# pytorch/QNNPACK

Hardware: AMD Instinct MI355X
Metric: q8gemm_int8_tops (higher is better)
Workload: dtype u8; 1 GPU; q8gemm M=N=K=4096 uint8 (qnnp_fully_connected_nc_q8, int8 MFMA, fused Q31 requantize); kernel=q8_gemm_mfma_256x256_c16, device=gfx950:sramecc+:xnack-, compute_units=256

## Files before the change

### qnnpack_amd/csrc/hip/q8gemm256x.hip

```cpp
#include <hip/hip_runtime.h>

#include <stdint.h>
#include <stdlib.h>

#include <type_traits>

#include "device_ops.hip.h"
#include "gemm256x_map.h"
#include "igemm_params.h"
#include "per_device.h"
#include "requant.hip.h"

namespace qnnp {

namespace {

namespace map = g256x;

constexpr int kBM = 256;
constexpr int kBN = 256;
constexpr int kBK = 64;
constexpr int kThreads = 512;
constexpr int kTM = 4;
constexpr int kTN = 8;
constexpr int kHalf = kTN / 2;
constexpr int kMma = kTM * kHalf;
static_assert(kBM == map::kRows && kBK == map::kTileK && kThreads == map::kWgThreads, "gemm256x_map.h describes this tile");

template <int P1, bool P2, int SYNC, bool MORE>
struct Tile {
  static constexpr int p1 = P1;
  static constexpr bool p2 = P2;
  static constexpr int sync = SYNC;
  static constexpr bool more = MORE;
};
constexpr int kSlotsEven = 0, kSlotsOdd = 1, kSlotsLiteral = 2;
using FirstTile = Tile<1, true, map::kFirstVmcnt, true>;
using SteadyTile = Tile<1, true, map::kSteadyVmcnt, true>;
template <bool ODD, uint32_t LEFT>
using DrainTile = Tile<map::p1_mode(ODD, LEFT), map::p2_issues(LEFT), map::sync_vmcnt(ODD, LEFT), LEFT != 1>;

template <int SEQ, int CLAMP, int SLOTS, int ABL = 0, bool ROWSUM = false, int OPT = 0>
__global__ __launch_bounds__(kThreads, 2)
void q8_gemm_mfma_256x256_c16_kernel(const IgemmParams p)
{
  static_assert(SEQ == kRqShift0Ofs || SEQ == kRqBoundedOfs || SEQ == kRqGeneral, "offset forms, or the general one");
  __shared__ __attribute__((aligned(16))) uint8_t lds[map::kLdsBytes];

  const uint32_t tid = threadIdx.x;
  const uint32_t lane = tid & 63u;
  const uint32_t wave = __builtin_amdgcn_readfirstlane(tid >> 6);
  const uint32_t wm = wave >> 1;
  const uint32_t wn = wave & 1u;
  const uint32_t g = blockIdx.y;
  QNNP_TRACE_WAVE04(p, lane, wave, 0);
  QNNP_TRACE_WAVE04_WALL(p, lane, wave, 0);

  const uint32_t tiles_m = (p.rows + kBM - 1) / kBM;
  const uint32_t tiles_n = p.n_pad / kBN;
  uint32_t m_tile, n_tile;
  {
    const uint32_t nwg = gridDim.x;
    const uint32_t xcd = blockIdx.x & 7u;
    const uint32_t idx = blockIdx.x >> 3;
    const uint32_t q = nwg >> 3, r = nwg & 7u;
    const uint32_t logical = xcd * q + min(xcd, r) + idx;
    constexpr uint32_t kBand = 4;
    const uint32_t band = p.tiles_n_magic != 0 ? __umulhi(logical >> 2, p.tiles_n_magic) : logical >> 2;
    const uint32_t within = logical - band * kBand * tiles_n;
    const uint32_t rows_in_band = min(kBand, tiles_m - band * kBand);
    if (rows_in_band == kBand) {
      m_tile = band * kBand + (within & 3u);
      n_tile = within >> 2;
    } else {
      m_tile = band * kBand + within % rows_in_band;
      n_tile = within / rows_in_band;
    }
  }

  const uint32_t nblocks = p.n_pad / 32;
  const uint32_t kblocks = p.k_pad / 32;
  const uint32_t ktiles = p.k_pad / kBK;
  const uint32_t nb0 = n_tile * (kBN / 32);

  const bool table_rows = p.offsets_dense != 0;
  const uint8_t* a_base = scalar_ptr(table_rows ? p.input + static_cast<uint64_t>(g) * p.kc
      : p.input + static_cast<uint64_t>(m_tile * kBM) * p.input_stride + static_cast<uint64_t>(g) * p.kc);
  uint32_t a_voff[map::kAPieces];
#pragma unroll
  for (uint32_t i = 0; i < map::kAPieces; i++) {
    const uint32_t m = map::a_clamp_row(m_tile * kBM + map::a_dma_row(i, tid), p.rows);
    a_voff[i] = (m - m_tile * kBM) * p.input_stride + map::a_dma_src(tid, false);
    if (table_rows) {
      const uint32_t img = p.rpi_magic != 0 ? __umulhi(m, p.rpi_magic) : m / p.rows_per_image;
      const uint32_t pix = m - img * p.rows_per_image;
      a_voff[i] = img * static_cast<uint32_t>(p.image_stride) + static_cast<uint32_t>(p.offsets[pix]) + map::a_dma_src(tid, false);
    }
  }
  const uint32_t a_half_back = map::a_dma_src(tid, false) - map::a_dma_src(tid, true);
  const uint8_t* w_base = scalar_ptr(reinterpret_cast<const uint8_t*>(p.packed_w) + static_cast<uint64_t>(g) * nblocks * kblocks * 1024 +
      (static_cast<uint64_t>(nb0 + (wave >> 1)) * kblocks + (wave & 1u)) * 1024);
  uint32_t w_voff[2];
#pragma unroll
  for (int i = 0; i < 2; i++) w_voff[i] = lane * 16 + static_cast<uint32_t>(i) * 4u * kblocks * 1024u;

  auto a_dst = [&](uint32_t piece, uint32_t slot) __attribute__((always_inline)) -> uint8_t* {
    return lds + map::kABase + slot * map::kPairBytes + map::a_dma_wave_dst(piece, wave);
  };
  auto w_dst = [&](uint32_t piece, uint32_t slot) __attribute__((always_inline)) -> uint8_t* {
    return lds + map::kWBase + slot * map::kWTileBytes + (piece * 8 + wave) * 1024;
  };
  auto a_src = [&](uint32_t pair) __attribute__((always_inline)) -> const uint8_t* {
    return a_base + static_cast<uint64_t>(pair) * map::kPairK;
  };
  auto w_src = [&](uint32_t kt) __attribute__((always_inline)) -> const uint8_t* {
    return w_base + static_cast<uint64_t>(kt) * 2048;
  };
  auto stage_pair = [&](uint32_t pair) __attribute__((always_inline)) {
#pragma unroll
    for (uint32_t piece = 0; piece < map::kAPieces; piece++) dma16_saddr(a_src(pair), a_voff[piece], a_dst(piece, map::a_slot(pair)));
  };
  auto stage_w = [&](uint32_t kt) __attribute__((always_inline)) {
#pragma unroll
    for (uint32_t piece = 0; piece < map::kWPieces; piece++) dma16_saddr(w_src(kt), w_voff[piece], w_dst(piece, map::w_slot(kt)));
  };

  stage_pair(0);
  stage_w(0);

  const int32_t* bias_tab = SEQ == kRqGeneral ? p.bias2 : p.bias2u;
  uint8_t* bias_line = lds + map::kBiasBase + wave * 512;
  if (lane < 32) {
    dma16_saddr(scalar_ptr(reinterpret_cast<const uint8_t*>(bias_tab + static_cast<uint64_t>(g) * p.n_pad + (nb0 + wn * 4) * 32)),
                   lane * 16, bias_line);
  }

  stage_pair(1);
  stage_w(1);
  stage_w(2);

  const uint32_t frow = lane & 15u;
  const uint32_t fg = lane >> 4;
  uint32_t a_off[2][2];
  uint32_t w_off;
#pragma unroll
  for (uint32_t h = 0; h < 2; h++) {
#pragma unroll
    for (uint32_t s2 = 0; s2 < 2; s2++) {
      a_off[h][s2] = map::kABase + map::a_lds_byte(map::a_frag_row(wm, 0, lane), map::a_frag_chunk(h, lane)) + s2 * 2 * map::kPairBytes;
      asm volatile("" : "+v"(a_off[h][s2]));
    }
  }
  w_off = map::kWBase + (wn * 8 + (fg >> 1)) * 1024 + (frow + 32 * (fg & 1u)) * 16;
  asm volatile("" : "+v"(w_off));
  v4i fa[kTM];
  v4i wl[kHalf], wh[kHalf];

  auto read_a = [&](auto known_c, uint32_t h, uint32_t slot, int tm) __attribute__((always_inline)) {
    const uint32_t imm = tm * 16 * map::kPairK;
    if constexpr (decltype(known_c)::value) {
      fa[tm] = *reinterpret_cast<const v4i*>(lds + a_off[h][slot >> 1] + (slot & 1u) * map::kPairBytes + imm);
    } else {
      fa[tm] = *reinterpret_cast<const v4i*>(lds + slot * map::kPairBytes + a_off[h][0] + imm);
    }
  };
  auto read_w = [&](auto known_c, uint32_t slot, int tn, v4i& dst) __attribute__((always_inline)) {
    const uint32_t imm = (tn >> 1) * 2048 + (tn & 1) * 256;
    dst = *reinterpret_cast<const v4i*>(lds + slot * map::kWTileBytes + w_off + imm);
  };

  const uint32_t flip = p.a_flip;
  uint32_t rs[kTM] = {0u, 0u, 0u, 0u};
  auto flip_half = [&](int tm, int half) __attribute__((always_inline)) {
    if constexpr (ROWSUM) {
      if (half) {
        rs[tm] = __builtin_amdgcn_sad_u8(static_cast<uint32_t>(fa[tm].z), 0u, rs[tm]);
        rs[tm] = __builtin_amdgcn_sad_u8(static_cast<uint32_t>(fa[tm].w), 0u, rs[tm]);
      } else {
        rs[tm] = __builtin_amdgcn_sad_u8(static_cast<uint32_t>(fa[tm].x), 0u, rs[tm]);
        rs[tm] = __builtin_amdgcn_sad_u8(static_cast<uint32_t>(fa[tm].y), 0u, rs[tm]);
      }
      asm volatile("" : "+v"(rs[tm]));
    }
    if constexpr ((ABL & 2) != 0) {
      asm volatile("" : "+v"(fa[tm]));
    } else if (half) {
      fa[tm].z ^= static_cast<int>(flip);
      fa[tm].w ^= static_cast<int>(flip);
      asm volatile("" : "+v"(fa[tm].z), "+v"(fa[tm].w));
    } else {
      fa[tm].x ^= static_cast<int>(flip);
      fa[tm].y ^= static_cast<int>(flip);
      asm volatile("" : "+v"(fa[tm].x), "+v"(fa[tm].y));
    }
  };

  v4i acc[kTM][kTN];
  auto mma = [&](const v4i& w, int tm, int tn) __attribute__((always_inline)) {
    if constexpr ((ABL & 4) != 0) return;
    acc[tm][tn] = __builtin_amdgcn_mfma_i32_16x16x64_i8(w, fa[tm], acc[tm][tn], 0, 0, 0);
  };

  wait_vmcnt<map::kPrologueVmcnt>();
  __builtin_amdgcn_s_barrier();
  QNNP_TRACE_WAVE04(p, lane, wave, 1);
  using T = std::true_type;
  using F = std::false_type;
#pragma unroll
  for (int tm = 0; tm < kTM; tm++) read_a(T{}, 0u, 0u, tm);
#pragma unroll
  for (int tn = 0; tn < kHalf; tn++) read_w(T{}, 0u, tn, wl[tn]);
#pragma unroll
  for (int tn = 0; tn < kTN; tn++) {
    const v4i b = *reinterpret_cast<const v4i*>(bias_line + tn * 64 + fg * 16);
#pragma unroll
    for (int tm = 0; tm < kTM; tm++) acc[tm][tn] = b;
  }
#pragma unroll
  for (int tm = 0; tm < 2; tm++) { flip_half(tm, 0); flip_half(tm, 1); }
  asm volatile("" : "+v"(wl[0]), "+v"(wl[1]), "+v"(wl[2]), "+v"(wl[3]));
  if constexpr ((ABL & 16) != 0) { wh[0] = wl[0]; wh[1] = wl[1]; wh[2] = wl[2]; wh[3] = wl[3]; }

  if constexpr ((OPT & 4) != 0) {
    if (wave >= 4) __builtin_amdgcn_s_setprio(1);
  }

  auto iteration = [&](auto tile_c, auto known_c, auto h_c, uint32_t kt, uint32_t ws, uint32_t as) __attribute__((always_inline)) {
    using TileT = decltype(tile_c);
    constexpr int P1 = (ABL & 8) != 0 ? 0 : TileT::p1;
    constexpr bool MORE = TileT::more;
    constexpr bool P2F = TileT::p2 && (ABL & 8) == 0;
    constexpr int SYNC = (ABL & 32) != 0 ? -1 : TileT::sync;
    constexpr bool KNOWN = decltype(known_c)::value;
    constexpr bool READS = (ABL & 16) == 0;
    constexpr uint32_t H = decltype(h_c)::value;
    const uint32_t ws_next = ws + 1 == map::kWSlots ? 0 : ws + 1;
    const uint32_t as_fill = as == 0 ? map::kASlots - 1 : as - 1;
    const uint32_t as_next = H == 0 ? as : (as + 1 == map::kASlots ? 0 : as + 1);
    auto a_piece_off = [&](uint32_t piece) __attribute__((always_inline)) -> uint32_t {
      return P1 == 2 ? a_voff[piece] - a_half_back : a_voff[piece];
    };

    QNNP_PIN();
#pragma unroll
    for (int i = 0; i < kMma; i++) {
      const int tm = i / kHalf, tn = ((OPT & 1) == 0 && (tm & 1) != 0) ? kHalf - 1 - i % kHalf : i % kHalf;
      if constexpr (P1 != 0 && KNOWN) {
        if (i % 8 == 0) { dma16_set_m0(a_dst(map::a_issue_piece(H, i / 8), as_fill)); QNNP_PIN(); }
      }
      mma(wl[tn], tm, tn);
      QNNP_PIN();
      if constexpr (READS) {
        if (i < kHalf) { read_w(known_c, ws, kHalf + i, wh[i]); QNNP_PIN(); }
      }
      if constexpr (P1 != 0 && KNOWN) {
        if (i % 8 == 0) { dma16_saddr_m0_set(a_src(map::a_issue_pair(kt)), a_piece_off(map::a_issue_piece(H, i / 8))); QNNP_PIN(); }
      } else if constexpr (P1 != 0) {
        if (i % 8 == 0) {
          dma16_saddr(a_src(map::a_issue_pair(kt)), a_piece_off(map::a_issue_piece(H, i / 8)), a_dst(map::a_issue_piece(H, i / 8), as_fill));
          QNNP_PIN();
        }
      }
      if (i == 2) { __builtin_amdgcn_s_waitcnt(0xC47F); QNNP_PIN(); }
      if (i == 2 || i == 3) { flip_half(2, i - 2); QNNP_PIN(); }
      if (i == 6) { __builtin_amdgcn_s_waitcnt(0xC47F); QNNP_PIN(); }
      if (i == 6 || i == 7) { flip_half(3, i - 6); QNNP_PIN(); }
      if (i == kMma - 2) { __builtin_amdgcn_s_waitcnt(0xC07F); QNNP_PIN(); }
    }
    asm volatile("" : "+v"(wh[0]), "+v"(wh[1]), "+v"(wh[2]), "+v"(wh[3]));
    QNNP_PIN();

    if constexpr (SYNC >= 0) {
      wait_vmcnt<SYNC>();
      __builtin_amdgcn_s_barrier();
    }
    QNNP_PIN();

#pragma unroll
    for (int i = 0; i < kMma; i++) {
      const int tm = i / kHalf, tn = ((OPT & 1) == 0 && (tm & 1) != 0) ? kHalf - 1 - i % kHalf : i % kHalf;
      if constexpr (P2F && KNOWN) {
        if (i % 8 == 0) { dma16_set_m0(w_dst(i / 8, ws)); QNNP_PIN(); }
      }
      mma(wh[tn], tm, kHalf + tn);
      QNNP_PIN();
      if constexpr (MORE && READS) {
        if (tm == 0) { read_w(known_c, ws_next, tn, wl[tn]); QNNP_PIN(); }
        if (i % kHalf == kHalf - 1) { read_a(known_c, 1u - H, as_next, tm); QNNP_PIN(); }
      }
      if constexpr (P2F && KNOWN) {
        if (i % 8 == 0) { dma16_saddr_m0_set(w_src(map::w_issue_tile(kt)), w_voff[i / 8]); QNNP_PIN(); }
      } else if constexpr (P2F) {
        if (i % 8 == 0) { dma16_saddr(w_src(map::w_issue_tile(kt)), w_voff[i / 8], w_dst(i / 8, ws)); QNNP_PIN(); }
      }
      if constexpr (MORE) {
        if (i == 9) { __builtin_amdgcn_s_waitcnt(0xC17F); QNNP_PIN(); }
        if (i == 9 || i == 10) { flip_half(0, i - 9); QNNP_PIN(); }
        if (i == 13) { __builtin_amdgcn_s_waitcnt(0xC17F); QNNP_PIN(); }
        if (i == 13 || i == 14) { flip_half(1, i - 13); QNNP_PIN(); }
      }
    }
    if constexpr (MORE) asm volatile("" : "+v"(wl[0]), "+v"(wl[1]), "+v"(wl[2]), "+v"(wl[3]));
    QNNP_PIN();
  };

  auto lit = [&](auto tile_c, auto x_c, uint32_t kt) __attribute__((always_inline)) {
    constexpr uint32_t X = decltype(x_c)::value;
    static_assert(X < map::kPeriod, "one ring period");
    iteration(tile_c, T{}, std::integral_constant<uint32_t, (X & 1u)>{}, kt, map::w_slot(X), map::a_slot(X >> 1));
  };
  using X0 = std::integral_constant<uint32_t, 0>;
  using X1 = std::integral_constant<uint32_t, 1>;
  using X2 = std::integral_constant<uint32_t, 2>;
  using X3 = std::integral_constant<uint32_t, 3>;
  using X4 = std::integral_constant<uint32_t, 4>;
  using X5 = std::integral_constant<uint32_t, 5>;

  lit(FirstTile{}, X0{}, 0u);
  QNNP_TRACE_WAVE04(p, lane, wave, 2);
  uint32_t kt = 1;
  if constexpr (SLOTS == kSlotsLiteral) {
    for (; kt + map::kPeriod + 4 + map::kDrain <= ktiles; kt += map::kPeriod) {
      lit(SteadyTile{}, X1{}, kt);
      lit(SteadyTile{}, X2{}, kt + 1);
      lit(SteadyTile{}, X3{}, kt + 2);
      lit(SteadyTile{}, X4{}, kt + 3);
      lit(SteadyTile{}, X5{}, kt + 4);
      lit(SteadyTile{}, X0{}, kt + 5);
    }
    lit(SteadyTile{}, X1{}, kt);
    lit(SteadyTile{}, X2{}, kt + 1);
    lit(SteadyTile{}, X3{}, kt + 2);
    lit(SteadyTile{}, X4{}, kt + 3);
    QNNP_TRACE_WAVE04(p, lane, wave, 3);
    lit(DrainTile<false, 5>{}, X5{}, kt + 4);
    lit(DrainTile<false, 4>{}, X0{}, kt + 5);
    lit(DrainTile<false, 3>{}, X1{}, kt + 6);
    QNNP_TRACE_WAVE04(p, lane, wave, 4);
    lit(DrainTile<false, 2>{}, X2{}, kt + 7);
    lit(DrainTile<false, 1>{}, X3{}, kt + 8);
  } else {
    uint32_t ws = 1, as = 0;
    using H0 = std::integral_constant<uint32_t, 0>;
    using H1 = std::integral_constant<uint32_t, 1>;
    auto odd_tile = [&](auto tile_c) __attribute__((always_inline)) {
      iteration(tile_c, F{}, H1{}, kt, ws, as);
      kt++;
      ws = ws + 1 == map::kWSlots ? 0 : ws + 1;
      as = as + 1 == map::kASlots ? 0 : as + 1;
    };
    auto even_tile = [&](auto tile_c) __attribute__((always_inline)) {
      iteration(tile_c, F{}, H0{}, kt, ws, as);
      kt++;
      ws = ws + 1 == map::kWSlots ? 0 : ws + 1;
    };
    while (kt + 1 + map::kDrain < ktiles) {
      odd_tile(SteadyTile{});
      even_tile(SteadyTile{});
    }
    QNNP_TRACE_WAVE04(p, lane, wave, 3);
    if constexpr (SLOTS == kSlotsOdd) {
      odd_tile(SteadyTile{});
      even_tile(DrainTile<true, 5>{});
      odd_tile(DrainTile<true, 4>{});
      even_tile(DrainTile<true, 3>{});
      odd_tile(DrainTile<true, 2>{});
      even_tile(DrainTile<true, 1>{});
    } else {
      odd_tile(DrainTile<false, 5>{});
      even_tile(DrainTile<false, 4>{});
      odd_tile(DrainTile<false, 3>{});
      even_tile(DrainTile<false, 2>{});
      odd_tile(DrainTile<false, 1>{});
    }
    QNNP_TRACE_WAVE04(p, lane, wave, 4);
  }
  QNNP_TRACE_WAVE04(p, lane, wave, 5);

  if constexpr ((ABL & 1) != 0) {
#pragma unroll
    for (int tm = 0; tm < kTM; tm++) {
#pragma unroll
      for (int tn = 0; tn < kTN; tn++) asm volatile("" : : "v"(acc[tm][tn]));
    }
    return;
  }
  const uint32_t m0 = m_tile * kBM + wm * 64;
  const uint32_t n0 = (nb0 + wn * 4) * 32;
  uint8_t* out0 = p.output + static_cast<uint64_t>(m0) * p.output_stride + static_cast<uint64_t>(g) * p.n + n0;
  const uint32_t st_row = frow & 7u;
  const uint32_t st_col = (frow >> 3) * 64 + fg * 16;
  const bool col_ok = n0 + st_col < p.n;
  auto transpose4 = [&](uint32_t (&q)[4]) __attribute__((always_inline)) {
    const auto s02 = __builtin_amdgcn_permlane32_swap(q[0], q[2], false, false);
    const auto s13 = __builtin_amdgcn_permlane32_swap(q[1], q[3], false, false);
    const auto lo = __builtin_amdgcn_permlane16_swap(s02[0], s13[0], false, false);
    const auto hi = __builtin_amdgcn_permlane16_swap(s02[1], s13[1], false, false);
    q[0] = lo[0]; q[1] = lo[1]; q[2] = hi[0]; q[3] = hi[1];
  };
#pragma unroll
  for (int tm = 0; tm < kTM; tm++) {
    if constexpr (ROWSUM) {
      uint32_t t = rs[tm];
      t += static_cast<uint32_t>(__shfl_xor(static_cast<int>(t), 16));
      t += static_cast<uint32_t>(__shfl_xor(static_cast<int>(t), 32));
      const uint32_t term = static_cast<uint32_t>(p.row_coeff) * (t - 128u * p.k_pad);
#pragma unroll
      for (int tn = 0; tn < kTN; tn++) {
#pragma unroll
        for (int r = 0; r < 4; r++) acc[tm][tn][r] = static_cast<int>(static_cast<uint32_t>(acc[tm][tn][r]) + term);
      }
    }
    uint32_t lo[4], hi[4];
#pragma unroll
    for (int j = 0; j < 4; j++) {
      lo[j] = q31_requantize_pack4_clamp<SEQ, CLAMP>(acc[tm][j][0], acc[tm][j][1], acc[tm][j][2], acc[tm][j][3], p.rq);
      hi[j] = q31_requantize_pack4_clamp<SEQ, CLAMP>(acc[tm][4 + j][0], acc[tm][4 + j][1], acc[tm][4 + j][2], acc[tm][4 + j][3], p.rq);
    }
    transpose4(lo);
    transpose4(hi);
    typedef int nt_v4i __attribute__((ext_vector_type(4)));
    nt_v4i x, y;
#pragma unroll
    for (int j = 0; j < 4; j++) {
      x[j] = __builtin_amdgcn_update_dpp(static_cast<int>(lo[j]), static_cast<int>(hi[j]), 0x128, 0xF, 0xC, false);
      y[j] = __builtin_amdgcn_update_dpp(static_cast<int>(hi[j]), static_cast<int>(lo[j]), 0x128, 0xF, 0x3, false);
    }
    const uint32_t rx = tm * 16 + st_row, ry = rx + 8;
    nt_v4i* dx = reinterpret_cast<nt_v4i*>(out0 + static_cast<uint64_t>(rx) * p.output_stride + st_col);
    nt_v4i* dy = reinterpret_cast<nt_v4i*>(out0 + static_cast<uint64_t>(ry) * p.output_stride + st_col);
    const bool stores = (ABL & 64) == 0 || p.rows == 0xFFFFFFFFu;
    if (m0 + rx < p.rows && col_ok && stores) {
      if (p.stream_out) asm volatile("global_store_dwordx4 %0, %1, off nt" : : "v"(dx), "v"(x) : "memory");
      else *dx = x;
    }
    if (m0 + ry < p.rows && col_ok && stores) {
      if (p.stream_out) asm volatile("global_store_dwordx4 %0, %1, off nt" : : "v"(dy), "v"(y) : "memory");
      else *dy = y;
    }
    if (tm == 1) QNNP_TRACE_WAVE04(p, lane, wave, 6);
  }
  QNNP_TRACE_WAVE04(p, lane, wave, 7);
#ifdef QNNP_ENABLE_ABLATION
  if (p.trace != nullptr) {
    wait_vmcnt<0>();
    QNNP_TRACE_WAVE04_WALL(p, lane, wave, 1);
  }
#endif
}
#undef QNNP_PIN

template <int SLOTS, bool ROWSUM>
int launch_x(const IgemmParams& p, const dim3& grid, hipStream_t stream)
{
  int rc = QNNP_HIP_EINVAL;
#ifdef QNNP_ENABLE_ABLATION
  if constexpr (SLOTS == kSlotsLiteral && !ROWSUM) {
    const char* env = getenv("QNNP_GFX950_ABLATE");
    const int abl = env != nullptr ? atoi(env) : 0;
#define QNNP_ABL_CASE(V) case V: hipLaunchKernelGGL((q8_gemm_mfma_256x256_c16_kernel<kRqShift0Ofs, 1, kSlotsLiteral, V>), grid, dim3(kThreads), 0, stream, p); \
        return launch_status();
    switch (abl) {
      QNNP_ABL_CASE(1) QNNP_ABL_CASE(2) QNNP_ABL_CASE(4) QNNP_ABL_CASE(8) QNNP_ABL_CASE(16) QNNP_ABL_CASE(24)
      QNNP_ABL_CASE(27) QNNP_ABL_CASE(32) QNNP_ABL_CASE(59) QNNP_ABL_CASE(64)
      default: break;
    }
#undef QNNP_ABL_CASE
    const char* oenv = getenv("QNNP_C16_OPT");
    if (oenv != nullptr && atoi(oenv) == 1) {
      hipLaunchKernelGGL((q8_gemm_mfma_256x256_c16_kernel<kRqShift0Ofs, 1, kSlotsLiteral, 0, false, 1>), grid, dim3(kThreads), 0, stream, p);
      return launch_status();
    }
    if (oenv != nullptr && atoi(oenv) == 4) {
      hipLaunchKernelGGL((q8_gemm_mfma_256x256_c16_kernel<kRqShift0Ofs, 1, kSlotsLiteral, 0, false, 4>), grid, dim3(kThreads), 0, stream, p);
      return launch_status();
    }
  }
#endif
  if (p.rq.f.shift != 0 && p.rq.f.bounded && p.rq.f.ofs_kind == 2 && !p.rq.full_range) {
    if (p.rq.zp_late == 0) hipLaunchKernelGGL((q8_gemm_mfma_256x256_c16_kernel<kRqBoundedOfs, 1, SLOTS, 0, ROWSUM>), grid, dim3(kThreads), 0, stream, p);
    else hipLaunchKernelGGL((q8_gemm_mfma_256x256_c16_kernel<kRqBoundedOfs, 2, SLOTS, 0, ROWSUM>), grid, dim3(kThreads), 0, stream, p);
    return launch_status();
  }
  requant_dispatch_ofs(p.rq, [&](auto seq, auto full) {
    constexpr int kSeq = decltype(seq)::value;
    if constexpr (decltype(full)::value) {
      hipLaunchKernelGGL((q8_gemm_mfma_256x256_c16_kernel<kSeq, 0, SLOTS, 0, ROWSUM>), grid, dim3(kThreads), 0, stream, p);
    } else if (p.rq.zp_late == 0) {
      hipLaunchKernelGGL((q8_gemm_mfma_256x256_c16_kernel<kSeq, 1, SLOTS, 0, ROWSUM>), grid, dim3(kThreads), 0, stream, p);
    } else {
      hipLaunchKernelGGL((q8_gemm_mfma_256x256_c16_kernel<kSeq, 2, SLOTS, 0, ROWSUM>), grid, dim3(kThreads), 0, stream, p);
    }
    rc = launch_status();
  });
  return rc;
}

}

int gemm256x_launch(const IgemmParams& p, uint32_t groups, hipStream_t stream, const char** name)
{
  const uint32_t tiles_m = (p.rows + kBM - 1) / kBM;
  const uint32_t tiles_n = p.n_pad / kBN;
  const dim3 grid(tiles_m * tiles_n, groups, 1);
  IgemmParams pm = p;
  pm.tiles_n_magic = tiles_n == 1 ? 0u : reciprocal_floor_plus1(tiles_n);
  const uint32_t ktiles = p.k_pad / kBK;
  const int slots = map::literal_slots(ktiles) ? kSlotsLiteral : (ktiles & 1u) != 0 ? kSlotsOdd : kSlotsEven;
  if (p.row_coeff != 0) {
    *name = "q8_gemm_mfma_256x256_r16";
    return slots == kSlotsLiteral ? launch_x<kSlotsLiteral, true>(pm, grid, stream)
         : slots == kSlotsOdd   ? launch_x<kSlotsOdd, true>(pm, grid, stream) : launch_x<kSlotsEven, true>(pm, grid, stream);
  }
  *name = "q8_gemm_mfma_256x256_c16";
  return slots == kSlotsLiteral ? launch_x<kSlotsLiteral, false>(pm, grid, stream)
       : slots == kSlotsOdd   ? launch_x<kSlotsOdd, false>(pm, grid, stream) : launch_x<kSlotsEven, false>(pm, grid, stream);
}

}
```

Baseline: 2816 TOPS.

## Split kernel arguments into hot/cold/table lines with explicit scalar loads

Replaces the IgemmParams kernel argument with a compact 192-byte struct laid out as a 64-byte hot header, a cold part and an offset table. Each part is fetched with explicit s_load instructions. The hot header is loaded up front; the cold part (output, requant params) is issued after the prologue DMAs and waited on later; the table is loaded only when indirect rows are used. The tile-index mapping replaces the modulo/divide path with a multiply-by-magic form. The goal is to cut kernel-entry scalar load latency and prologue stalls, at the cost of hand-written asm that must stay in sync with the struct layout.

```diff
diff --git a/qnnpack_amd/csrc/hip/gemm256x_args.h b/qnnpack_amd/csrc/hip/gemm256x_args.h
--- /dev/null
+++ b/qnnpack_amd/csrc/hip/gemm256x_args.h
@@ -0,0 +1,96 @@
+#pragma once
+
+#include <stddef.h>
+#include <stdint.h>
+
+#include "igemm_params.h"
+
+namespace qnnp {
+
+struct Gemm256xHot {
+  const uint8_t* input;
+  const int8_t* packed_w;
+  const int32_t* bias;
+  uint32_t rows;
+  uint32_t input_stride;
+  uint32_t kc;
+  uint32_t n_pad;
+  uint32_t k_pad;
+  uint32_t tiles_n_magic;
+  uint32_t offsets_dense;
+  uint32_t reserved[3];
+};
+
+struct Gemm256xCold {
+  unsigned long long* trace;
+  uint8_t* output;
+  uint32_t output_stride;
+  uint32_t n;
+  uint32_t a_flip;
+  int32_t row_coeff;
+  uint32_t stream_out;
+  uint32_t reserved;
+  RequantDev rq;
+};
+
+struct Gemm256xTable {
+  const int32_t* offsets;
+  uint32_t rows_per_image;
+  uint32_t image_stride;
+  uint32_t rpi_magic;
+  uint32_t reserved;
+};
+
+struct alignas(64) Gemm256xArgs {
+  Gemm256xHot hot;
+  Gemm256xCold cold;
+  Gemm256xTable table;
+};
+
+constexpr size_t kGemm256xHotBytes = 64;
+constexpr size_t kGemm256xColdBytes = 104;
+constexpr size_t kGemm256xTableBytes = 24;
+static_assert(sizeof(Gemm256xHot) == kGemm256xHotBytes, "the hot header is one 64-byte line");
+static_assert(sizeof(Gemm256xCold) == kGemm256xColdBytes && sizeof(Gemm256xTable) == kGemm256xTableBytes, "whole scalar loads: 16 + 8 + 2 and 4 + 2 dwords");
+static_assert(offsetof(Gemm256xArgs, hot) == 0 && offsetof(Gemm256xArgs, cold) == kGemm256xHotBytes &&
+              offsetof(Gemm256xArgs, table) == kGemm256xHotBytes + kGemm256xColdBytes, "hot header first, the cold part right behind it, then the table");
+static_assert(sizeof(Gemm256xArgs) == 192 && alignof(Gemm256xArgs) == 64, "three lines");
+static_assert(offsetof(Gemm256xCold, trace) == 0, "a stamp build loads `trace` at the cold part's first byte");
+
+inline bool gemm256x_offset_form(const RequantDev& rq)
+{
+  return rq.f.shift == 0 || (rq.f.bounded != 0 && (rq.full_range != 0 || rq.f.ofs_kind == 2));
+}
+
+inline Gemm256xArgs gemm256x_make_args(const IgemmParams& p, uint32_t tiles_n_magic)
+{
+  Gemm256xArgs a;
+  a.hot.input = p.input;
+  a.hot.packed_w = p.packed_w;
+  a.hot.bias = gemm256x_offset_form(p.rq) ? p.bias2u : p.bias2;
+  a.hot.rows = p.rows;
+  a.hot.input_stride = p.input_stride;
+  a.hot.kc = p.kc;
+  a.hot.n_pad = p.n_pad;
+  a.hot.k_pad = p.k_pad;
+  a.hot.tiles_n_magic = tiles_n_magic;
+  a.hot.offsets_dense = p.offsets_dense;
+  a.hot.reserved[0] = a.hot.reserved[1] = a.hot.reserved[2] = 0;
+  a.cold.trace = p.trace;
+  a.cold.output = p.output;
+  a.cold.output_stride = p.output_stride;
+  a.cold.n = p.n;
+  a.cold.a_flip = p.a_flip;
+  a.cold.row_coeff = p.row_coeff;
+  a.cold.stream_out = p.stream_out;
+  a.cold.reserved = 0;
+  a.cold.rq = p.rq;
+  a.table.offsets = p.offsets;
+  a.table.rows_per_image = p.rows_per_image;
+  a.table.image_stride = static_cast<uint32_t>(p.image_stride);
+  a.table.rpi_magic = p.rpi_magic;
+  a.table.reserved = 0;
+  return a;
+}
+
+}
diff --git a/qnnpack_amd/csrc/hip/q8gemm256x.hip b/qnnpack_amd/csrc/hip/q8gemm256x.hip
--- a/qnnpack_amd/csrc/hip/q8gemm256x.hip
+++ b/qnnpack_amd/csrc/hip/q8gemm256x.hip
@@ -6,6 +6,7 @@
 #include <type_traits>
 
 #include "device_ops.hip.h"
+#include "gemm256x_args.h"
 #include "gemm256x_map.h"
 #include "igemm_params.h"
 #include "per_device.h"
@@ -40,27 +41,115 @@
 template <bool ODD, uint32_t LEFT>
 using DrainTile = Tile<map::p1_mode(ODD, LEFT), map::p2_issues(LEFT), map::sync_vmcnt(ODD, LEFT), LEFT != 1>;
 
+typedef uint32_t hot_words __attribute__((ext_vector_type(16)));
+static_assert(sizeof(hot_words) == sizeof(Gemm256xHot), "one s_load_dwordx16");
+
+struct TraceArg {
+  unsigned long long* trace;
+};
+
+__device__ __forceinline__ Gemm256xHot fetch_hot_header(TraceArg& tp)
+{
+  const auto* kernarg = __builtin_amdgcn_kernarg_segment_ptr();
+  hot_words w;
+#ifdef QNNP_ENABLE_ABLATION
+  uint64_t trace;
+  asm volatile("s_load_dwordx16 %0, %2, 0x0\n\ts_load_dwordx2 %1, %2, 0x40\n\ts_waitcnt lgkmcnt(0)" : "=&s"(w), "=&s"(trace) : "s"(kernarg));
+  tp.trace = reinterpret_cast<unsigned long long*>(trace);
+#else
+  asm volatile("s_load_dwordx16 %0, %1, 0x0\n\ts_waitcnt lgkmcnt(0)" : "=&s"(w) : "s"(kernarg));
+  tp.trace = nullptr;
+#endif
+  auto ptr = [&](int i) __attribute__((always_inline)) { return (static_cast<uint64_t>(w[i + 1]) << 32) | w[i]; };
+  static_assert(offsetof(Gemm256xHot, input) == 0 && offsetof(Gemm256xHot, packed_w) == 8 && offsetof(Gemm256xHot, bias) == 16 &&
+                offsetof(Gemm256xHot, rows) == 24 && offsetof(Gemm256xHot, input_stride) == 28 && offsetof(Gemm256xHot, kc) == 32 &&
+                offsetof(Gemm256xHot, n_pad) == 36 && offsetof(Gemm256xHot, k_pad) == 40 && offsetof(Gemm256xHot, tiles_n_magic) == 44 &&
+                offsetof(Gemm256xHot, offsets_dense) == 48, "the words below");
+  Gemm256xHot h;
+  h.input = reinterpret_cast<const uint8_t*>(ptr(0));
+  h.packed_w = reinterpret_cast<const int8_t*>(ptr(2));
+  h.bias = reinterpret_cast<const int32_t*>(ptr(4));
+  h.rows = w[6];
+  h.input_stride = w[7];
+  h.kc = w[8];
+  h.n_pad = w[9];
+  h.k_pad = w[10];
+  h.tiles_n_magic = w[11];
+  h.offsets_dense = w[12];
+  return h;
+}
+
+struct ColdWords {
+  hot_words a;
+  uint32_t b __attribute__((ext_vector_type(8)));
+  uint32_t c __attribute__((ext_vector_type(2)));
+};
+static_assert(kGemm256xColdBytes == 64 + 32 + 8, "the three loads below");
+
+__device__ __forceinline__ void fetch_cold_issue(ColdWords& w)
+{
+  const auto* kernarg = __builtin_amdgcn_kernarg_segment_ptr();
+  asm volatile("s_load_dwordx16 %0, %3, 0x40\n\ts_load_dwordx8 %1, %3, 0x80\n\ts_load_dwordx2 %2, %3, 0xa0"
+               : "=&s"(w.a), "=&s"(w.b), "=&s"(w.c) : "s"(kernarg));
+  static_assert(kGemm256xHotBytes == 0x40, "the offsets above");
+}
+
+__device__ __forceinline__ Gemm256xCold fetch_cold_wait(ColdWords& w)
+{
+  asm volatile("s_waitcnt lgkmcnt(0)" : "+s"(w.a), "+s"(w.b), "+s"(w.c));
+  uint32_t words[kGemm256xColdBytes / 4];
+#pragma unroll
+  for (int i = 0; i < 16; i++) words[i] = w.a[i];
+#pragma unroll
+  for (int i = 0; i < 8; i++) words[16 + i] = w.b[i];
+  words[24] = w.c[0];
+  words[25] = w.c[1];
+  Gemm256xCold c;
+  __builtin_memcpy(&c, words, sizeof(c));
+  return c;
+}
+
+__device__ __forceinline__ Gemm256xTable fetch_table()
+{
+  const auto* kernarg = __builtin_amdgcn_kernarg_segment_ptr();
+  uint32_t lo __attribute__((ext_vector_type(4)));
+  uint32_t hi __attribute__((ext_vector_type(2)));
+  asm volatile("s_load_dwordx4 %0, %2, 0xa8\n\ts_load_dwordx2 %1, %2, 0xb8\n\ts_waitcnt lgkmcnt(0)" : "=&s"(lo), "=&s"(hi) : "s"(kernarg));
+  static_assert(kGemm256xHotBytes + kGemm256xColdBytes == 0xa8 && kGemm256xTableBytes == 24, "the offsets above");
+  static_assert(offsetof(Gemm256xTable, offsets) == 0 && offsetof(Gemm256xTable, rows_per_image) == 8 &&
+                offsetof(Gemm256xTable, image_stride) == 12 && offsetof(Gemm256xTable, rpi_magic) == 16, "the words below");
+  Gemm256xTable t;
+  t.offsets = reinterpret_cast<const int32_t*>((static_cast<uint64_t>(lo[1]) << 32) | lo[0]);
+  t.rows_per_image = lo[2];
+  t.image_stride = lo[3];
+  t.rpi_magic = hi[0];
+  t.reserved = 0;
+  return t;
+}
+
 template <int SEQ, int CLAMP, int SLOTS, int ABL = 0, bool ROWSUM = false, int OPT = 0>
 __global__ __launch_bounds__(kThreads, 2)
-void q8_gemm_mfma_256x256_c16_kernel(const IgemmParams p)
+void q8_gemm_mfma_256x256_c16_kernel(const Gemm256xArgs a)
 {
   static_assert(SEQ == kRqShift0Ofs || SEQ == kRqBoundedOfs || SEQ == kRqGeneral, "offset forms, or the general one");
   __shared__ __attribute__((aligned(16))) uint8_t lds[map::kLdsBytes];
 
+  [[maybe_unused]] TraceArg tp;
+  const Gemm256xHot p = fetch_hot_header(tp);
   const uint32_t tid = threadIdx.x;
   const uint32_t lane = tid & 63u;
   const uint32_t wave = __builtin_amdgcn_readfirstlane(tid >> 6);
   const uint32_t wm = wave >> 1;
   const uint32_t wn = wave & 1u;
   const uint32_t g = blockIdx.y;
-  QNNP_TRACE_WAVE04(p, lane, wave, 0);
-  QNNP_TRACE_WAVE04_WALL(p, lane, wave, 0);
+  QNNP_TRACE_WAVE04(tp, lane, wave, 0);
+  QNNP_TRACE_WAVE04_WALL(tp, lane, wave, 0);
 
   const uint32_t tiles_m = (p.rows + kBM - 1) / kBM;
   const uint32_t tiles_n = p.n_pad / kBN;
   uint32_t m_tile, n_tile;
   {
-    const uint32_t nwg = gridDim.x;
+    const uint32_t nwg = tiles_m * tiles_n;
     const uint32_t xcd = blockIdx.x & 7u;
     const uint32_t idx = blockIdx.x >> 3;
     const uint32_t q = nwg >> 3, r = nwg & 7u;
@@ -69,13 +158,9 @@
     const uint32_t band = p.tiles_n_magic != 0 ? __umulhi(logical >> 2, p.tiles_n_magic) : logical >> 2;
     const uint32_t within = logical - band * kBand * tiles_n;
     const uint32_t rows_in_band = min(kBand, tiles_m - band * kBand);
-    if (rows_in_band == kBand) {
-      m_tile = band * kBand + (within & 3u);
-      n_tile = within >> 2;
-    } else {
-      m_tile = band * kBand + within % rows_in_band;
-      n_tile = within / rows_in_band;
-    }
+    const uint32_t third = __umulhi(within, 0xAAAAAAABu) >> 1;
+    n_tile = rows_in_band == 3 ? third : within >> (rows_in_band >> 1);
+    m_tile = band * kBand + (within - n_tile * rows_in_band);
   }
 
   const uint32_t nblocks = p.n_pad / 32;
@@ -87,15 +172,35 @@
   const uint8_t* a_base = scalar_ptr(table_rows ? p.input + static_cast<uint64_t>(g) * p.kc
       : p.input + static_cast<uint64_t>(m_tile * kBM) * p.input_stride + static_cast<uint64_t>(g) * p.kc);
   uint32_t a_voff[map::kAPieces];
+  uint32_t a_row[map::kAPieces];
 #pragma unroll
   for (uint32_t i = 0; i < map::kAPieces; i++) {
-    const uint32_t m = map::a_clamp_row(m_tile * kBM + map::a_dma_row(i, tid), p.rows);
-    a_voff[i] = (m - m_tile * kBM) * p.input_stride + map::a_dma_src(tid, false);
-    if (table_rows) {
-      const uint32_t img = p.rpi_magic != 0 ? __umulhi(m, p.rpi_magic) : m / p.rows_per_image;
-      const uint32_t pix = m - img * p.rows_per_image;
-      a_voff[i] = img * static_cast<uint32_t>(p.image_stride) + static_cast<uint32_t>(p.offsets[pix]) + map::a_dma_src(tid, false);
-    }
+    a_row[i] = map::a_clamp_row(m_tile * kBM + map::a_dma_row(i, tid), p.rows);
+    a_voff[i] = (a_row[i] - m_tile * kBM) * p.input_stride + map::a_dma_src(tid, false);
+  }
+  if (table_rows) {
+    const Gemm256xTable table = fetch_table();
+    const uint32_t rpi = table.rows_per_image;
+    const uint32_t rpi_magic = table.rpi_magic;
+    const uint32_t image_stride = table.image_stride;
+    const int32_t* offsets = table.offsets;
+    uint32_t img[map::kAPieces], ofs[map::kAPieces];
+    if (rpi_magic != 0) {
+#pragma unroll
+      for (uint32_t i = 0; i < map::kAPieces; i++) img[i] = __umulhi(a_row[i], rpi_magic);
+    } else {
+#pragma unroll
+      for (uint32_t i = 0; i < map::kAPieces; i++) img[i] = a_row[i] / rpi;
+    }
+#pragma unroll
+    for (uint32_t i = 0; i < map::kAPieces; i++) {
+      const uint32_t pix = a_row[i] - img[i] * rpi;
+      asm volatile("global_load_dword %0, %1, %2" : "=v"(ofs[i]) : "v"(pix * 4u), "s"(offsets) : "memory");
+    }
+    asm volatile("s_waitcnt vmcnt(0)" : "+v"(ofs[0]), "+v"(ofs[1]), "+v"(ofs[2]), "+v"(ofs[3]) : : "memory");
+    static_assert(map::kAPieces == 4, "the wait above names four entries");
+#pragma unroll
+    for (uint32_t i = 0; i < map::kAPieces; i++) a_voff[i] = img[i] * image_stride + ofs[i] + map::a_dma_src(tid, false);
   }
   const uint32_t a_half_back = map::a_dma_src(tid, false) - map::a_dma_src(tid, true);
   const uint8_t* w_base = scalar_ptr(reinterpret_cast<const uint8_t*>(p.packed_w) + static_cast<uint64_t>(g) * nblocks * kblocks * 1024 +
@@ -128,7 +233,7 @@
   stage_pair(0);
   stage_w(0);
 
-  const int32_t* bias_tab = SEQ == kRqGeneral ? p.bias2 : p.bias2u;
+  const int32_t* bias_tab = p.bias;
   uint8_t* bias_line = lds + map::kBiasBase + wave * 512;
   if (lane < 32) {
     dma16_saddr(scalar_ptr(reinterpret_cast<const uint8_t*>(bias_tab + static_cast<uint64_t>(g) * p.n_pad + (nb0 + wn * 4) * 32)),
@@ -138,6 +243,9 @@
   stage_pair(1);
   stage_w(1);
   stage_w(2);
+
+  ColdWords cold_words;
+  fetch_cold_issue(cold_words);
 
   const uint32_t frow = lane & 15u;
   const uint32_t fg = lane >> 4;
@@ -169,7 +277,8 @@
     dst = *reinterpret_cast<const v4i*>(lds + slot * map::kWTileBytes + w_off + imm);
   };
 
-  const uint32_t flip = p.a_flip;
+  const Gemm256xCold cold = fetch_cold_wait(cold_words);
+  const uint32_t flip = cold.a_flip;
   uint32_t rs[kTM] = {0u, 0u, 0u, 0u};
   auto flip_half = [&](int tm, int half) __attribute__((always_inline)) {
     if constexpr (ROWSUM) {
@@ -203,7 +312,7 @@
 
   wait_vmcnt<map::kPrologueVmcnt>();
   __builtin_amdgcn_s_barrier();
-  QNNP_TRACE_WAVE04(p, lane, wave, 1);
+  QNNP_TRACE_WAVE04(tp, lane, wave, 1);
   using T = std::true_type;
   using F = std::false_type;
 #pragma unroll
@@ -317,7 +426,7 @@
   using X5 = std::integral_constant<uint32_t, 5>;
 
   lit(FirstTile{}, X0{}, 0u);
-  QNNP_TRACE_WAVE04(p, lane, wave, 2);
+  QNNP_TRACE_WAVE04(tp, lane, wave, 2);
   uint32_t kt = 1;
   if constexpr (SLOTS == kSlotsLiteral) {
     for (; kt + map::kPeriod + 4 + map::kDrain <= ktiles; kt += map::kPeriod) {
@@ -332,11 +441,11 @@
     lit(SteadyTile{}, X2{}, kt + 1);
     lit(SteadyTile{}, X3{}, kt + 2);
     lit(SteadyTile{}, X4{}, kt + 3);
-    QNNP_TRACE_WAVE04(p, lane, wave, 3);
+    QNNP_TRACE_WAVE04(tp, lane, wave, 3);
     lit(DrainTile<false, 5>{}, X5{}, kt + 4);
     lit(DrainTile<false, 4>{}, X0{}, kt + 5);
     lit(DrainTile<false, 3>{}, X1{}, kt + 6);
-    QNNP_TRACE_WAVE04(p, lane, wave, 4);
+    QNNP_TRACE_WAVE04(tp, lane, wave, 4);
     lit(DrainTile<false, 2>{}, X2{}, kt + 7);
     lit(DrainTile<false, 1>{}, X3{}, kt + 8);
   } else {
@@ -358,7 +467,7 @@
       odd_tile(SteadyTile{});
       even_tile(SteadyTile{});
     }
-    QNNP_TRACE_WAVE04(p, lane, wave, 3);
+    QNNP_TRACE_WAVE04(tp, lane, wave, 3);
     if constexpr (SLOTS == kSlotsOdd) {
       odd_tile(SteadyTile{});
       even_tile(DrainTile<true, 5>{});
@@ -373,9 +482,9 @@
       even_tile(DrainTile<false, 2>{});
       odd_tile(DrainTile<false, 1>{});
     }
-    QNNP_TRACE_WAVE04(p, lane, wave, 4);
-  }
-  QNNP_TRACE_WAVE04(p, lane, wave, 5);
+    QNNP_TRACE_WAVE04(tp, lane, wave, 4);
+  }
+  QNNP_TRACE_WAVE04(tp, lane, wave, 5);
 
   if constexpr ((ABL & 1) != 0) {
 #pragma unroll
@@ -387,10 +496,10 @@
   }
   const uint32_t m0 = m_tile * kBM + wm * 64;
   const uint32_t n0 = (nb0 + wn * 4) * 32;
-  uint8_t* out0 = p.output + static_cast<uint64_t>(m0) * p.output_stride + static_cast<uint64_t>(g) * p.n + n0;
+  uint8_t* out0 = cold.output + static_cast<uint64_t>(m0) * cold.output_stride + static_cast<uint64_t>(g) * cold.n + n0;
   const uint32_t st_row = frow & 7u;
   const uint32_t st_col = (frow >> 3) * 64 + fg * 16;
-  const bool col_ok = n0 + st_col < p.n;
+  const bool col_ok = n0 + st_col < cold.n;
   auto transpose4 = [&](uint32_t (&q)[4]) __attribute__((always_inline)) {
     const auto s02 = __builtin_amdgcn_permlane32_swap(q[0], q[2], false, false);
     const auto s13 = __builtin_amdgcn_permlane32_swap(q[1], q[3], false, false);
@@ -404,7 +513,7 @@
       uint32_t t = rs[tm];
       t += static_cast<uint32_t>(__shfl_xor(static_cast<int>(t), 16));
       t += static_cast<uint32_t>(__shfl_xor(static_cast<int>(t), 32));
-      const uint32_t term = static_cast<uint32_t>(p.row_coeff) * (t - 128u * p.k_pad);
+      const uint32_t term = static_cast<uint32_t>(cold.row_coeff) * (t - 128u * p.k_pad);
 #pragma unroll
       for (int tn = 0; tn < kTN; tn++) {
 #pragma unroll
@@ -414,8 +523,8 @@
     uint32_t lo[4], hi[4];
 #pragma unroll
     for (int j = 0; j < 4; j++) {
-      lo[j] = q31_requantize_pack4_clamp<SEQ, CLAMP>(acc[tm][j][0], acc[tm][j][1], acc[tm][j][2], acc[tm][j][3], p.rq);
-      hi[j] = q31_requantize_pack4_clamp<SEQ, CLAMP>(acc[tm][4 + j][0], acc[tm][4 + j][1], acc[tm][4 + j][2], acc[tm][4 + j][3], p.rq);
+      lo[j] = q31_requantize_pack4_clamp<SEQ, CLAMP>(acc[tm][j][0], acc[tm][j][1], acc[tm][j][2], acc[tm][j][3], cold.rq);
+      hi[j] = q31_requantize_pack4_clamp<SEQ, CLAMP>(acc[tm][4 + j][0], acc[tm][4 + j][1], acc[tm][4 + j][2], acc[tm][4 + j][3], cold.rq);
     }
     transpose4(lo);
     transpose4(hi);
@@ -427,38 +536,50 @@
       y[j] = __builtin_amdgcn_update_dpp(static_cast<int>(hi[j]), static_cast<int>(lo[j]), 0x128, 0xF, 0x3, false);
     }
     const uint32_t rx = tm * 16 + st_row, ry = rx + 8;
-    nt_v4i* dx = reinterpret_cast<nt_v4i*>(out0 + static_cast<uint64_t>(rx) * p.output_stride + st_col);
-    nt_v4i* dy = reinterpret_cast<nt_v4i*>(out0 + static_cast<uint64_t>(ry) * p.output_stride + st_col);
+    nt_v4i* dx = reinterpret_cast<nt_v4i*>(out0 + static_cast<uint64_t>(rx) * cold.output_stride + st_col);
+    nt_v4i* dy = reinterpret_cast<nt_v4i*>(out0 + static_cast<uint64_t>(ry) * cold.output_stride + st_col);
     const bool stores = (ABL & 64) == 0 || p.rows == 0xFFFFFFFFu;
     if (m0 + rx < p.rows && col_ok && stores) {
-      if (p.stream_out) asm volatile("global_store_dwordx4 %0, %1, off nt" : : "v"(dx), "v"(x) : "memory");
+      if (cold.stream_out) asm volatile("global_store_dwordx4 %0, %1, off nt" : : "v"(dx), "v"(x) : "memory");
       else *dx = x;
     }
     if (m0 + ry < p.rows && col_ok && stores) {
-      if (p.stream_out) asm volatile("global_store_dwordx4 %0, %1, off nt" : : "v"(dy), "v"(y) : "memory");
+      if (cold.stream_out) asm volatile("global_store_dwordx4 %0, %1, off nt" : : "v"(dy), "v"(y) : "memory");
       else *dy = y;
     }
-    if (tm == 1) QNNP_TRACE_WAVE04(p, lane, wave, 6);
-  }
-  QNNP_TRACE_WAVE04(p, lane, wave, 7);
+    if (tm == 1) QNNP_TRACE_WAVE04(tp, lane, wave, 6);
+  }
+  QNNP_TRACE_WAVE04(tp, lane, wave, 7);
 #ifdef QNNP_ENABLE_ABLATION
-  if (p.trace != nullptr) {
+  if (tp.trace != nullptr) {
     wait_vmcnt<0>();
-    QNNP_TRACE_WAVE04_WALL(p, lane, wave, 1);
+    QNNP_TRACE_WAVE04_WALL(tp, lane, wave, 1);
   }
 #endif
 }
 #undef QNNP_PIN
 
+template <int SEQ, int CLAMP, int SLOTS, bool ROWSUM>
+int launch_one(const Gemm256xArgs& a, const dim3& grid, hipStream_t stream)
+{
+  if (gemm256x_offset_form(a.cold.rq) != (SEQ != kRqGeneral)) return QNNP_HIP_EINVAL;
+  hipLaunchKernelGGL((q8_gemm_mfma_256x256_c16_kernel<SEQ, CLAMP, SLOTS, 0, ROWSUM>), grid, dim3(kThreads), 0, stream, a);
+  return launch_status();
+}
+
 template <int SLOTS, bool ROWSUM>
-int launch_x(const IgemmParams& p, const dim3& grid, hipStream_t stream)
-{
+int launch_x(const IgemmParams& p, uint32_t tiles_n_magic, const dim3& grid, hipStream_t stream)
+{
+  const Gemm256xArgs a = gemm256x_make_args(p, tiles_n_magic);
+  const RequantDev& rq = a.cold.rq;
   int rc = QNNP_HIP_EINVAL;
 #ifdef QNNP_ENABLE_ABLATION
   if constexpr (SLOTS == kSlotsLiteral && !ROWSUM) {
+    Gemm256xArgs ab = a;
+    ab.hot.bias = p.bias2u;
     const char* env = getenv("QNNP_GFX950_ABLATE");
     const int abl = env != nullptr ? atoi(env) : 0;
-#define QNNP_ABL_CASE(V) case V: hipLaunchKernelGGL((q8_gemm_mfma_256x256_c16_kernel<kRqShift0Ofs, 1, kSlotsLiteral, V>), grid, dim3(kThreads), 0, stream, p); \
+#define QNNP_ABL_CASE(V) case V: hipLaunchKernelGGL((q8_gemm_mfma_256x256_c16_kernel<kRqShift0Ofs, 1, kSlotsLiteral, V>), grid, dim3(kThreads), 0, stream, ab); \
         return launch_status();
     switch (abl) {
       QNNP_ABL_CASE(1) QNNP_ABL_CASE(2) QNNP_ABL_CASE(4) QNNP_ABL_CASE(8) QNNP_ABL_CASE(16) QNNP_ABL_CASE(24)
@@ -468,30 +589,27 @@
 #undef QNNP_ABL_CASE
     const char* oenv = getenv("QNNP_C16_OPT");
     if (oenv != nullptr && atoi(oenv) == 1) {
-      hipLaunchKernelGGL((q8_gemm_mfma_256x256_c16_kernel<kRqShift0Ofs, 1, kSlotsLiteral, 0, false, 1>), grid, dim3(kThreads), 0, stream, p);
+      hipLaunchKernelGGL((q8_gemm_mfma_256x256_c16_kernel<kRqShift0Ofs, 1, kSlotsLiteral, 0, false, 1>), grid, dim3(kThreads), 0, stream, ab);
       return launch_status();
     }
     if (oenv != nullptr && atoi(oenv) == 4) {
-      hipLaunchKernelGGL((q8_gemm_mfma_256x256_c16_kernel<kRqShift0Ofs, 1, kSlotsLiteral, 0, false, 4>), grid, dim3(kThreads), 0, stream, p);
+      hipLaunchKernelGGL((q8_gemm_mfma_256x256_c16_kernel<kRqShift0Ofs, 1, kSlotsLiteral, 0, false, 4>), grid, dim3(kThreads), 0, stream, ab);
       return launch_status();
     }
   }
 #endif
-  if (p.rq.f.shift != 0 && p.rq.f.bounded && p.rq.f.ofs_kind == 2 && !p.rq.full_range) {
-    if (p.rq.zp_late == 0) hipLaunchKernelGGL((q8_gemm_mfma_256x256_c16_kernel<kRqBoundedOfs, 1, SLOTS, 0, ROWSUM>), grid, dim3(kThreads), 0, stream, p);
-    else hipLaunchKernelGGL((q8_gemm_mfma_256x256_c16_kernel<kRqBoundedOfs, 2, SLOTS, 0, ROWSUM>), grid, dim3(kThreads), 0, stream, p);
-    return launch_status();
-  }
-  requant_dispatch_ofs(p.rq, [&](auto seq, auto full) {
+  if (rq.f.shift != 0 && rq.f.bounded && rq.f.ofs_kind == 2 && !rq.full_range) {
+    return rq.zp_late == 0 ? launch_one<kRqBoundedOfs, 1, SLOTS, ROWSUM>(a, grid, stream) : launch_one<kRqBoundedOfs, 2, SLOTS, ROWSUM>(a, grid, stream);
+  }
+  requant_dispatch_ofs(rq, [&](auto seq, auto full) {
     constexpr int kSeq = decltype(seq)::value;
     if constexpr (decltype(full)::value) {
-      hipLaunchKernelGGL((q8_gemm_mfma_256x256_c16_kernel<kSeq, 0, SLOTS, 0, ROWSUM>), grid, dim3(kThreads), 0, stream, p);
-    } else if (p.rq.zp_late == 0) {
-      hipLaunchKernelGGL((q8_gemm_mfma_256x256_c16_kernel<kSeq, 1, SLOTS, 0, ROWSUM>), grid, dim3(kThreads), 0, stream, p);
+      rc = launch_one<kSeq, 0, SLOTS, ROWSUM>(a, grid, stream);
+    } else if (rq.zp_late == 0) {
+      rc = launch_one<kSeq, 1, SLOTS, ROWSUM>(a, grid, stream);
     } else {
-      hipLaunchKernelGGL((q8_gemm_mfma_256x256_c16_kernel<kSeq, 2, SLOTS, 0, ROWSUM>), grid, dim3(kThreads), 0, stream, p);
-    }
-    rc = launch_status();
+      rc = launch_one<kSeq, 2, SLOTS, ROWSUM>(a, grid, stream);
+    }
   });
   return rc;
 }
@@ -503,18 +621,17 @@
   const uint32_t tiles_m = (p.rows + kBM - 1) / kBM;
   const uint32_t tiles_n = p.n_pad / kBN;
   const dim3 grid(tiles_m * tiles_n, groups, 1);
-  IgemmParams pm = p;
-  pm.tiles_n_magic = tiles_n == 1 ? 0u : reciprocal_floor_plus1(tiles_n);
+  const uint32_t magic = tiles_n == 1 ? 0u : reciprocal_floor_plus1(tiles_n);
   const uint32_t ktiles = p.k_pad / kBK;
   const int slots = map::literal_slots(ktiles) ? kSlotsLiteral : (ktiles & 1u) != 0 ? kSlotsOdd : kSlotsEven;
   if (p.row_coeff != 0) {
     *name = "q8_gemm_mfma_256x256_r16";
-    return slots == kSlotsLiteral ? launch_x<kSlotsLiteral, true>(pm, grid, stream)
-         : slots == kSlotsOdd   ? launch_x<kSlotsOdd, true>(pm, grid, stream) : launch_x<kSlotsEven, true>(pm, grid, stream);
+    return slots == kSlotsLiteral ? launch_x<kSlotsLiteral, true>(p, magic, grid, stream)
+         : slots == kSlotsOdd   ? launch_x<kSlotsOdd, true>(p, magic, grid, stream) : launch_x<kSlotsEven, true>(p, magic, grid, stream);
   }
   *name = "q8_gemm_mfma_256x256_c16";
-  return slots == kSlotsLiteral ? launch_x<kSlotsLiteral, false>(pm, grid, stream)
-       : slots == kSlotsOdd   ? launch_x<kSlotsOdd, false>(pm, grid, stream) : launch_x<kSlotsEven, false>(pm, grid, stream);
-}
-
-}
+  return slots == kSlotsLiteral ? launch_x<kSlotsLiteral, false>(p, magic, grid, stream)
+       : slots == kSlotsOdd   ? launch_x<kSlotsOdd, false>(p, magic, grid, stream) : launch_x<kSlotsEven, false>(p, magic, grid, stream);
+}
+
+}
```

Result: slower. 2750 TOPS (-2.3%).
